# akashsengupta1997/STRAPS-3DHumanShapePose

Hardware: AMD Instinct MI355X
Metric: bodies/sec (higher is better)
Workload: dtype fp32 (encoder convolutions as exact bf16x3 operand splits (six bf16 products per term); in-step SMPL blend contraction and skinning as 3-product fp16 splits (fp16x3_lbs: 22-bit operands); fp32 accumulate throughout)

## Files before the change

straps-3dhumanshapepose_amd/csrc/backward.hip:

```cpp
#include "common.h"
#include <stdlib.h>

namespace {

struct WgradP {
    const float* x;
    const float* dy;
    float* part;
    int B, H, W, Cin, Cout, R, S, stride, pad, Ho, Wo;
    int M, rows_per_split, ct, it;
};

__device__ __attribute__((aligned(16))) float k_zero16w[4] = {0.f, 0.f, 0.f, 0.f};

template <int BCO, int BCI>
__global__ __launch_bounds__(256) void conv_wgrad_kernel(WgradP p) {
    constexpr int STG = 32 * (BCO + BCI);
    constexpr int LPD = BCO / 4, PWD = 64 / LPD, RDD = 8 / PWD;
    constexpr int LPX = BCI / 4, PWX = 64 / LPX, RDX = 8 / PWX;
    constexpr int MI = BCO / 64, NI = BCI / 64;
    extern __shared__ __attribute__((aligned(16))) float smem[];
    const int tid = threadIdx.x, lane = tid & 63, wave = tid >> 6;
    const int wave_u = __builtin_amdgcn_readfirstlane(wave);
    const int wm = wave >> 1, wn = wave & 1;
// ... 477 lines not shown
    const int cbeg = blockIdx.y * p.chunks_per_split;
    const int cend = min(cbeg + p.chunks_per_split, p.nchunks);
    const u16* zsrc = reinterpret_cast<const u16*>(k_zero16x);
    asm volatile("" : "+s"(zsrc));

    const int lp = (tid & 255) >> 3, ls = tid & 7;
    const int d_g = ls ^ (((lp >> 1) & 1) << 2);
    long long d_off[DR];
#pragma unroll
    for (int q = 0; q < DR; ++q) {
        const int px = lp + 32 * q;
        d_off[q] = ((long long)((co0 >> 5) + (d_g >> 2)) * p.rows + (px >> p.cw_log2) * p.W + (px & (p.cw - 1))) * 32 + (d_g & 3) * 8;
    }
    int x_pr[XR], x_pc[XR];
    long long x_g[XR];
#pragma unroll
    for (int q = 0; q < XR; ++q) {
        const int pp = lp + 32 * q;
        x_pr[q] = pp / pw - 1;
        x_pc[q] = pp - (x_pr[q] + 1) * pw - 1;
        const int g = ls ^ (((pp >> 1) & 1) << 2);
        x_g[q] = (long long)((ci0 >> 5) + (g >> 2)) * p.rows * 32 + (g & 3) * 8;
    }
    auto dma_chunk = [&](int c, int stage) {
        const int per_img = p.chunk_rows_per_img * p.chunks_per_row;
        const int b = c / per_img;
        const int rem = c - b * per_img;
        const int cr = rem / p.chunks_per_row, cc = rem - cr * p.chunks_per_row;
        const int ho0 = cr * p.rpc, wo0 = cc * p.cw;
        u16* D = smem + stage * STAGE;
        u16* X = D + 3 * DPX * 64;
        const u16* dbase = p.dy3 + ((long long)(b * p.H + ho0) * p.W + wo0) * 32;
        const u16* xsrc = p.x3 + ((long long)(b * p.H + ho0) * p.W + wo0) * 32;
#pragma unroll
        for (int q = 0; q < DR; ++q) {
            if (NG > 1 && (q & 1) != grp) continue;
#pragma unroll
            for (int pl = 0; pl < 3; ++pl)
                __builtin_amdgcn_global_load_lds((const __attribute__((address_space(1))) void*)(dbase + d_off[q] + pl * p.dps),
                                                 (__attribute__((address_space(3))) void*)(D + (pl * DPX + 32 * q + 8 * wave_u) * 64), 16, 0, 0);
        }
#pragma unroll
        for (int q = 0; q < XR; ++q) {
            if (q * 32 + 8 * wave_u >= npatch || q * 32 + 8 * wave_u >= XPX) break;
            if (NG > 1 && ((q + DR) & 1) != grp) continue;
            const int hi = ho0 + x_pr[q], wi = wo0 + x_pc[q];
            const bool ok = (unsigned)hi < (unsigned)p.H && (unsigned)wi < (unsigned)p.W;
            const u16* src = ok ? xsrc + (x_pr[q] * p.W + x_pc[q]) * 32 + x_g[q] : zsrc;
            const long long ps = ok ? p.xps : 0;
#pragma unroll
            for (int pl = 0; pl < 3; ++pl)
                __builtin_amdgcn_global_load_lds((const __attribute__((address_space(1))) void*)(src + pl * ps),
                                                 (__attribute__((address_space(3))) void*)(X + (pl * XPX + 32 * q + 8 * wave_u) * 64), 16, 0, 0);
        }
    };

    const int t = lane & 15, ch16 = (lane >> 4) & 1, kh = lane >> 5;
    auto row_off = [&](int slot_px, int c4) {
        const int g = (c4 >> 3) ^ (((slot_px >> 1) & 1) << 2);
        return slot_px * 64 + g * 8 + (c4 & 4);
    };
    int d_fo[KSG][2], x_fo[KSG][2];
#pragma unroll
    for (int ks = 0; ks < KSG; ++ks)
#pragma unroll
        for (int r = 0; r < 2; ++r) {
            const int px = (grp + NG * ks) * 16 + kh * 8 + r * 4 + (t >> 2);
            d_fo[ks][r] = row_off(px, wm * 32 + ch16 * 16 + (t & 3) * 4);
            x_fo[ks][r] = (px >> p.cw_log2) * pw + (px & (p.cw - 1));
        }
    const int x_c4 = wn * 32 + ch16 * 16 + (t & 3) * 4;

    f32x16 acc[9];
#pragma unroll
    for (int tp = 0; tp < 9; ++tp)
#pragma unroll
        for (int q = 0; q < 16; ++q) acc[tp][q] = 0.f;
    if (cbeg < cend) dma_chunk(cbeg, 0);
    constexpr int TA[6] = {1, 0, 2, 0, 1, 0};
    constexpr int TB[6] = {1, 2, 0, 1, 0, 0};
    for (int c = cbeg; c < cend; ++c) {
        const int stage = (c - cbeg) & 1;
        asm volatile("s_waitcnt vmcnt(0)" ::: "memory");
        __builtin_amdgcn_s_barrier();
        asm volatile("" ::: "memory");
        if (c + 1 < cend && !(ABL & 1)) dma_chunk(c + 1, stage ^ 1);
        const u16* D = smem + ((ABL & 1) ? 0 : stage) * STAGE;
        const u16* X = D + 3 * DPX * 64;
        __builtin_amdgcn_s_setprio(1);
#pragma unroll
        for (int ks = 0; ks < KSG; ++ks) {
            bf16x8w a[3];
#pragma unroll
            for (int pl = 0; pl < 3; ++pl) a[pl] = tr_frag(D + pl * DPX * 64 + d_fo[ks][0], D + pl * DPX * 64 + d_fo[ks][1]);
#pragma unroll
            for (int tp0 = 0; tp0 < 9; tp0 += W3X_TG) {
                bf16x8w b[W3X_TG][3];
#pragma unroll
                for (int u = 0; u < W3X_TG; ++u) {
                    const int tp = tp0 + u;
                    if (tp >= 9) break;
                    const int sh = (ABL & 4) ? 0 : (tp / 3) * pw + (tp % 3);
                    const int o0 = row_off(x_fo[ks][0] + sh, x_c4), o1 = row_off(x_fo[ks][1] + sh, x_c4);
#pragma unroll
                    for (int pl = 0; pl < 3; ++pl) b[u][pl] = tr_frag(X + pl * XPX * 64 + o0, X + pl * XPX * 64 + o1);
                }
                if (ABL & 2) {
#pragma unroll
                    for (int u = 0; u < W3X_TG; ++u)
                        if (tp0 + u < 9)
#pragma unroll
                            for (int pl = 0; pl < 3; ++pl) acc[0][pl] += (float)b[u][pl][0] + (float)a[pl][1];
                    continue;
                }
#pragma unroll
                for (int e = 0; e < 6; ++e)
#pragma unroll
                    for (int u = 0; u < W3X_TG; ++u)
                        if (tp0 + u < 9) acc[tp0 + u] = __builtin_amdgcn_mfma_f32_32x32x16_bf16(a[TA[e]], b[u][TB[e]], acc[tp0 + u], 0, 0, 0);
            }
        }
        __builtin_amdgcn_s_setprio(0);
    }
    if constexpr (NG > 1) {
        float* R = smem_f + ((wave * 3) * 16) * 64 + lane;
#pragma unroll
        for (int rd = 0; rd < 3; ++rd) {
            __syncthreads();
            if (grp == 1) {
#pragma unroll
                for (int tp = 0; tp < 3; ++tp)
#pragma unroll
                    for (int q = 0; q < 16; ++q) R[(tp * 16 + q) * 64] = acc[rd * 3 + tp][q];
            }
            __syncthreads();
            if (grp == 0) {
#pragma unroll
                for (int tp = 0; tp < 3; ++tp)
#pragma unroll
                    for (int q = 0; q < 16; ++q) acc[rd * 3 + tp][q] += R[(tp * 16 + q) * 64];
            }
        }
        if (grp != 0) return;
    }
    const int i = lane & 31;
    float* o = p.part + (long long)blockIdx.y * p.Cout * 9 * p.Cin;
#pragma unroll
    for (int tp = 0; tp < 9; ++tp)
#pragma unroll
        for (int q = 0; q < 16; ++q) {
            const int co = co0 + wm * 32 + mfma_row(q, lane);
            o[((long long)co * 9 + tp) * p.Cin + ci0 + wn * 32 + i] = acc[tp][q];
        }
}

__global__ __launch_bounds__(256) void wgrad_reduce_kernel(const float* __restrict__ part, float* __restrict__ dw, int splits,
                                                           int Cout, int Cin, int RS, int accumulate) {
    __shared__ f32x4 red[4][64];
    const long long n = (long long)Cout * RS * Cin;
    const int lane = threadIdx.x & 63, sg = threadIdx.x >> 6;
    const long long idx = ((long long)blockIdx.x * 64 + lane) * 4;
    f32x4 s = {0.f, 0.f, 0.f, 0.f};
    int k = sg;
    for (; k + 12 < splits; k += 16) {
        const f32x4 v0 = *reinterpret_cast<const f32x4*>(part + (long long)k * n + idx);
        const f32x4 v1 = *reinterpret_cast<const f32x4*>(part + (long long)(k + 4) * n + idx);
        const f32x4 v2 = *reinterpret_cast<const f32x4*>(part + (long long)(k + 8) * n + idx);
        const f32x4 v3 = *reinterpret_cast<const f32x4*>(part + (long long)(k + 12) * n + idx);
        s += (v0 + v1) + (v2 + v3);
    }
    for (; k < splits; k += 4) s += *reinterpret_cast<const f32x4*>(part + (long long)k * n + idx);
    red[sg][lane] = s;
    __syncthreads();
    if (sg != 0) return;
    s = (red[0][lane] + red[1][lane]) + (red[2][lane] + red[3][lane]);
    const int ci = (int)(idx % Cin);
    long long t = idx / Cin;
    const int tap = (int)(t % RS);
    const int co = (int)(t / RS);
#pragma unroll
    for (int e = 0; e < 4; ++e) {
        const long long o = ((long long)co * Cin + ci + e) * RS + tap;
        dw[o] = accumulate ? dw[o] + s[e] : s[e];
    }
}

constexpr int TY = 2, TX = 32, PH = 2 * TY + 5, PW = 72, TPIX = TY * TX;
constexpr int CG = 4, GK = CG * 49, GNB = (GK + 31) / 32, GUNITS = 2 * GNB, UPW = (GUNITS + 3) / 4;

__global__ __launch_bounds__(256) void stem_tileact_kernel(const unsigned* __restrict__ nzmask, uint8_t* __restrict__ tact, int C, int H, int W,
                                                           int tiles_x, int tiles_y, int ntiles, int groups) {
    const int idx = blockIdx.x * 256 + threadIdx.x;
    if (idx >= ntiles * groups) return;
    const int grp = idx / ntiles, tile = idx - grp * ntiles;
    int bid = tile;
    const int b = bid / (tiles_x * tiles_y);
    bid -= b * tiles_x * tiles_y;
    const int ty = bid / tiles_x, tx = bid - ty * tiles_x;
    const int hi0 = 2 * (ty * TY) - 3, wi0 = 2 * (tx * TX) - 3;
    const int HC = (H + 3) >> 2, WW = (W + 255) >> 8;
    const int rc0 = max(hi0, 0) >> 2, rc1 = min(hi0 + PH - 1, H - 1) >> 2;
    const int wa = max(wi0 - 1, 0), wb = min(wi0 - 2 + PW, W - 1);
    const int c0 = grp * CG, nc = min(CG, C - c0);
    unsigned chact = 0;
    for (int cl = 0; cl < nc; ++cl) {
        unsigned any = 0;
        for (int rcell = rc0; rcell <= rc1; ++rcell)
            for (int word = wa >> 8; word <= (wb >> 8); ++word) {
                const int lo = max(wa, word << 8), hi = min(wb, (word << 8) + 255);
                const int b0 = (lo >> 3) & 31, b1 = (hi >> 3) & 31;
                const unsigned bits = (b1 == 31 ? 0xffffffffu : ((1u << (b1 + 1)) - 1u)) & ~((1u << b0) - 1u);
                any |= nzmask[(((long long)b * C + c0 + cl) * HC + rcell) * WW + word] & bits;
            }
        if (any) chact |= 1u << cl;
    }
    tact[idx] = (uint8_t)chact;
}

__global__ __launch_bounds__(256) void stem_tileany_kernel(const unsigned* __restrict__ nzmask, uint8_t* __restrict__ tany, int C, int H, int W,
                                                           int tiles_x, int tiles_y, int ntiles) {
    const int lane = threadIdx.x & 63, sub = lane & 31;
    const int tile = (blockIdx.x * 256 + threadIdx.x) >> 5;
    unsigned any = 0;
    if (tile < ntiles) {
        int bid = tile;
        const int b = bid / (tiles_x * tiles_y);
        bid -= b * tiles_x * tiles_y;
        const int ty = bid / tiles_x, tx = bid - ty * tiles_x;
        const int hi0 = 2 * (ty * TY) - 3, wi0 = 2 * (tx * TX) - 3;
        const int HC = (H + 3) >> 2, WW = (W + 255) >> 8;
        const int rc0 = max(hi0, 0) >> 2, rc1 = min(hi0 + PH - 1, H - 1) >> 2;
        const int wa = max(wi0 - 1, 0), wb = min(wi0 - 2 + PW, W - 1);
        for (int c = sub; c < C; c += 32)
            for (int rcell = rc0; rcell <= rc1; ++rcell)
                for (int word = wa >> 8; word <= (wb >> 8); ++word) {
                    const int lo = max(wa, word << 8), hi = min(wb, (word << 8) + 255);
                    const int b0 = (lo >> 3) & 31, b1 = (hi >> 3) & 31;
                    const unsigned bits = (b1 == 31 ? 0xffffffffu : ((1u << (b1 + 1)) - 1u)) & ~((1u << b0) - 1u);
                    any |= nzmask[(((long long)b * C + c) * HC + rcell) * WW + word] & bits;
                }
    }
    const unsigned long long bal = __ballot(any != 0u);
    const unsigned mine = (unsigned)(bal >> (lane & 32));
    if (sub == 0 && tile < ntiles) tany[tile] = mine ? 1 : 0;
}

__global__ __launch_bounds__(256) void stem_wgrad_kernel(const float* __restrict__ x, const float* __restrict__ dy,
                                                         float* __restrict__ part, const uint8_t* __restrict__ tact, int B, int C, int H,
                                                         int W, int Ho, int Wo,
                                                         int tiles_x, int tiles_y, int Kp, int ntiles, int rot) {
    __shared__ __attribute__((aligned(16))) float patch[2 * CG * PH * PW];
    __shared__ __attribute__((aligned(16))) float dys[2 * TPIX * 68];
    const int tid = threadIdx.x, lane = tid & 63;
    const int wave = __builtin_amdgcn_readfirstlane(tid >> 6);
    const int i = lane & 31, h = lane >> 5;
    const int c0 = blockIdx.y * CG;
    const int nc = min(CG, C - c0);
    const int gk = nc * 49;

    int u_a[UPW], u_nb[UPW], u_ko[UPW];
    unsigned u_span[UPW];
#pragma unroll
    for (int j = 0; j < UPW; ++j) {
        const int u = wave + 4 * j;
        u_a[j] = u & 1;
        u_nb[j] = u >> 1;
        const int k = u_nb[j] * 32 + i;
        int o = 0;
        if (u < GUNITS && k < gk) {
            const int cl = k / 49, rs = k - cl * 49;
            const int r = rs / 7, s_ = rs - r * 7;
            o = (cl * PH + r) * PW + s_ + 1;
        }
        u_ko[j] = o;
        const int k0 = u_nb[j] * 32;
        u_span[j] = 0;
        if (u < GUNITS && k0 < gk) {
            const int cl0 = k0 / 49, cl1 = min(k0 + 31, gk - 1) / 49;
            u_span[j] = (1u << cl0) | (1u << cl1);
        }
    }
    f32x16 acc[UPW];
#pragma unroll
    for (int j = 0; j < UPW; ++j)
#pragma unroll
        for (int q = 0; q < 16; ++q) acc[j][q] = 0.f;

    constexpr int PIT = (CG * PH * (PW / 4) + 255) / 256;
    constexpr int DIT = TPIX * 16 / 256;
    const bool vec = (W & 3) == 0;
    f32x4 pv[PIT], dv[DIT];
    auto tile_origin = [&](int tile, int& b, int& y0, int& x0) {
        b = tile / (tiles_x * tiles_y);
        const int bid = tile - b * tiles_x * tiles_y;
        const int ty = bid / tiles_x;
        y0 = ty * TY;
        x0 = (bid - ty * tiles_x) * TX;
    };
    auto issue_loads = [&](int tile, unsigned chact) {
        int b, y0, x0;
        tile_origin(tile, b, y0, x0);
        const int hi0 = 2 * y0 - 3, wi0 = 2 * x0 - 3;
#pragma unroll
        for (int it = 0; it < PIT; ++it) {
            const int idx = tid + it * 256;
            const int q = idx % (PW / 4);
// ... 608 lines not shown
int straps_internal_wgrad_reduce(const float* part, float* dw_oihw, int splits, int cout, int cin, int taps, int accumulate, hipStream_t st) {
    const long long n = (long long)cout * taps * cin;
    hipLaunchKernelGGL(wgrad_reduce_kernel, dim3((unsigned)(n / 256)), dim3(256), 0, st, part, dw_oihw, splits, cout, cin, taps, accumulate);
    STRAPS_CHECK_LAUNCH("wgrad_reduce_kernel");
    return STRAPS_OK;
}

static bool wgrad3_plan(int batch, int h, int w, int cin, int cout, int kh, int kw, int stride, int pad, Wgrad3P* p, int* splits, int cp = 32) {
    if (!(kh == 3 && kw == 3 && stride == 1 && pad == 1)) return false;
    if (w < 8 || (w & (w - 1)) != 0) return false;
    const int cw = w < 32 ? w : 32, rpc = cp / cw;
    if (h % rpc != 0) return false;
    int lg = 0;
    while ((1 << lg) < cw) ++lg;
    p->H = h; p->W = w; p->Cin = cin; p->Cout = cout; p->cw = cw; p->cw_log2 = lg; p->rpc = rpc;
    p->chunks_per_row = w / cw;
    p->chunk_rows_per_img = h / rpc;
    p->nchunks = batch * p->chunk_rows_per_img * p->chunks_per_row;
    p->it = cin / 64;
    const int tiles = (cout / 64) * (cin / 64);
    constexpr int W3_TARGET = 256;
    int s = (W3_TARGET + tiles - 1) / tiles;
    const int max_s = (p->nchunks + 3) / 4;
    if (s > max_s) s = max_s;
    if (s < 1) s = 1;
    p->chunks_per_split = (p->nchunks + s - 1) / s;
    *splits = (p->nchunks + p->chunks_per_split - 1) / p->chunks_per_split;
    return true;
}

extern "C" size_t straps_conv_wgrad_workspace_bytes(int batch, int h, int w, int cin, int cout, int kh, int kw, int stride, int pad) {
    Wgrad3P p3;
    int splits3;
    if (wgrad3_plan(batch, h, w, cin, cout, kh, kw, stride, pad, &p3, &splits3)) return (size_t)splits3 * cout * 9 * cin * sizeof(float);
    const int ho = (h + 2 * pad - kh) / stride + 1, wo = (w + 2 * pad - kw) / stride + 1;
    const long long M = (long long)batch * ho * wo;
    const bool big = wgrad_big_tile(M, cin, cout, kh * kw);
    const int tile = big ? 128 : 64;
    const int tiles = kh * kw * (cout / tile) * (cin / tile);
    return (size_t)wgrad_splits(M, tiles, big) * cout * kh * kw * cin * sizeof(float);
}

extern "C" int straps_conv_wgrad(const float* x, const float* dy, float* dw_oihw, void* workspace, int batch, int h, int w, int cin,
                                 int cout, int kh, int kw, int stride, int pad, int accumulate, void* stream) {
    STRAPS_REQUIRE(x && dy && dw_oihw && workspace, "straps_conv_wgrad: null pointer");
    STRAPS_REQUIRE(cin % 64 == 0 && cout % 64 == 0, "straps_conv_wgrad: need cin%%64==0 and cout%%64==0 (cin=%d cout=%d)", cin, cout);
    {
        Wgrad3P p3;
        int splits3;
        if (wgrad3_plan(batch, h, w, cin, cout, kh, kw, stride, pad, &p3, &splits3)) {
            p3.x = x; p3.dy = dy; p3.part = (float*)workspace;
            constexpr int NG3 = 2;
            const size_t lds = (size_t)NG3 * 2 * W3PX * 64 * sizeof(float);
            STRAPS_RAISE_LDS((conv_wgrad3x3_kernel<NG3>), lds, "conv_wgrad3x3_kernel");
            hipStream_t st3 = (hipStream_t)stream;
            hipLaunchKernelGGL(conv_wgrad3x3_kernel<NG3>, dim3((cout / 64) * (cin / 64), splits3), dim3(256 * NG3), lds, st3, p3);
            STRAPS_CHECK_LAUNCH("conv_wgrad3x3_kernel");
            const long long n3 = (long long)cout * 9 * cin;
            hipLaunchKernelGGL(wgrad_reduce_kernel, dim3((unsigned)(n3 / 256)), dim3(256), 0, st3, p3.part, dw_oihw, splits3, cout, cin, 9, accumulate);
            STRAPS_CHECK_LAUNCH("wgrad_reduce_kernel");
            return STRAPS_OK;
        }
    }
    WgradP p;
    p.x = x; p.dy = dy; p.part = (float*)workspace;
    p.B = batch; p.H = h; p.W = w; p.Cin = cin; p.Cout = cout; p.R = kh; p.S = kw; p.stride = stride; p.pad = pad;
    p.Ho = (h + 2 * pad - kh) / stride + 1;
    p.Wo = (w + 2 * pad - kw) / stride + 1;
    const long long M = (long long)batch * p.Ho * p.Wo;
    STRAPS_REQUIRE(M < (1LL << 31), "straps_conv_wgrad: problem too large");
    p.M = (int)M;
    const bool big = wgrad_big_tile(M, cin, cout, kh * kw);
    const int tile = big ? 128 : 64;
    p.ct = cout / tile; p.it = cin / tile;
    const int tiles = kh * kw * p.ct * p.it;
    const int splits = wgrad_splits(M, tiles, big);
    p.rows_per_split = (int)(((M + splits - 1) / splits + 31) / 32 * 32);
    hipStream_t st = (hipStream_t)stream;
    if (big) {
        STRAPS_RAISE_LDS((conv_wgrad_kernel<128, 128>), 64 * 1024, "conv_wgrad_kernel");
        hipLaunchKernelGGL((conv_wgrad_kernel<128, 128>), dim3(tiles, splits), dim3(256), 64 * 1024, st, p);
    } else {
        hipLaunchKernelGGL((conv_wgrad_kernel<64, 64>), dim3(tiles, splits), dim3(256), 32 * 1024, st, p);
    }
    STRAPS_CHECK_LAUNCH("conv_wgrad_kernel");
    const long long n = (long long)cout * kh * kw * cin;
    hipLaunchKernelGGL(wgrad_reduce_kernel, dim3((unsigned)(n / 256)), dim3(256), 0, st, p.part, dw_oihw, splits, cout, cin, kh * kw, accumulate);
    STRAPS_CHECK_LAUNCH("wgrad_reduce_kernel");
    return STRAPS_OK;
}

static int stem_wgrad_blocks(int ntiles) {
    static const int cap = STRAPS_TOOL_ENV_INT("STRAPS_STEM_WGRAD_BLOCKS", 256);
    return ntiles < cap ? ntiles : cap;
}

static int wgrad_x3_route(int batch, int h, int w, int cin, int cout, int kh, int kw, int stride, int pad) {
    Wgrad3P p3;
    int splits3;
    if (wgrad3_plan(batch, h, w, cin, cout, kh, kw, stride, pad, &p3, &splits3)) return 1;
    static const bool tap_x3 = !STRAPS_TOOL_ENV_INT("STRAPS_WGRAD_TAP_FP32", 0);
    return tap_x3 && (kh * kw > 1 || (cin >= 128 && cout >= 128)) ? 2 : 0;
}

static void wgrad_x3_block(long long M, int cin, int cout, int taps, bool big, int stride, int* bco, int* bci) {
    const int v = STRAPS_TOOL_ENV_INT("STRAPS_WGRAD_TILE", 0);
    if (v) {
        const int o = v / 1000, i = v % 1000;
        const bool known = (o == 256 && i == 64) || (o == 64 && i == 256) || (o == 256 && i == 128) || (o == 128 && i == 256) || (o == 128 && i == 64) ||
                           (o == 64 && i == 128) || (o == 128 && i == 128) || (o == 64 && i == 64);
        if (known && cout % o == 0 && cin % i == 0 && !(o == 128 && i == 128 && !big)) { *bco = o; *bci = i; }
        return;
    }
    if (taps == 1) {
        if (M >= 32768 && cout % 256 == 0 && cin % 128 == 0) { *bco = 256; *bci = 128; }
        else if (M <= 8192 && cout % 128 == 0 && cin % 128 == 0) {
            if (stride == 1 && cout > cin) { *bco = 64; *bci = 128; }
            else { *bco = 128; *bci = 64; }
        }
    } else if (cout % 256 == 0 && cin % 128 == 0) { *bco = 256; *bci = 128; }
    else if (cout % 128 == 0 && cin % 64 == 0) { *bco = 128; *bci = 64; }
}

extern "C" int straps_conv_wgrad_x3_on_planes(int batch, int h, int w, int cin, int cout, int kh, int kw, int stride, int pad) {
    return wgrad_x3_route(batch, h, w, cin, cout, kh, kw, stride, pad) != 0;
}

extern "C" int straps_conv_wgrad_x3(const float* x, const float* dy, const unsigned short* x3, long long x_plane_stride, const unsigned short* dy3,
                                    long long dy_plane_stride, float* dw_oihw, void* workspace, int batch, int h, int w, int cin, int cout, int kh,
                                    int kw, int stride, int pad, int accumulate, void* stream) {
    STRAPS_REQUIRE(dw_oihw && workspace, "straps_conv_wgrad_x3: null pointer");
    const int route = (x3 && dy3) ? wgrad_x3_route(batch, h, w, cin, cout, kh, kw, stride, pad) : 0;
    STRAPS_REQUIRE(route != 0 || (x && dy), "straps_conv_wgrad_x3: this shape runs on the fp32 tensors, which are NULL (see straps_conv_wgrad_x3_on_planes)");
    STRAPS_REQUIRE(cin % 64 == 0 && cout % 64 == 0, "straps_conv_wgrad_x3: need cin%%64==0 and cout%%64==0 (cin=%d cout=%d)", cin, cout);
    Wgrad3P p3;
    int splits3;
    if (route == 1 && wgrad3_plan(batch, h, w, cin, cout, kh, kw, stride, pad, &p3, &splits3)) {
        STRAPS_REQUIRE(x_plane_stride % 8 == 0 && dy_plane_stride % 8 == 0, "straps_conv_wgrad_x3: plane strides must be multiples of 8 elements");
        Wgrad3XP q;
        q.x3 = x3; q.dy3 = dy3; q.xps = x_plane_stride; q.dps = dy_plane_stride; q.part = (float*)workspace;
        q.H = p3.H; q.W = p3.W; q.Cin = p3.Cin; q.Cout = p3.Cout; q.cw = p3.cw; q.cw_log2 = p3.cw_log2; q.rpc = p3.rpc;
        q.chunks_per_row = p3.chunks_per_row; q.chunk_rows_per_img = p3.chunk_rows_per_img; q.nchunks = p3.nchunks;
        q.chunks_per_split = p3.chunks_per_split; q.it = p3.it;
        q.rows = (long long)batch * h * w;
        constexpr int W3X_NG = 2;
        hipStream_t st3 = (hipStream_t)stream;
        Wgrad3P p64;
        int splits64;
        const bool c64 = wgrad3_plan(batch, h, w, cin, cout, kh, kw, stride, pad, &p64, &splits64, 64) && splits64 <= splits3;
        if (c64) {
            q.rpc = p64.rpc; q.chunks_per_row = p64.chunks_per_row; q.chunk_rows_per_img = p64.chunk_rows_per_img; q.nchunks = p64.nchunks;
            q.chunks_per_split = p64.chunks_per_split;
            splits3 = splits64;
            const size_t lds = (size_t)2 * 3 * (64 + 136) * 64 * sizeof(u16);
            const dim3 grid3((cout / 64) * (cin / 64), splits3);
#ifdef STRAPS_TOOLS
            static const int abl = STRAPS_TOOL_ENV_INT("STRAPS_WGRAD3_ABL", 0);
            if (abl) {
                auto kern = abl == 1 ? conv_wgrad3x3_x3_kernel<W3X_NG, 64, 1> : abl == 2 ? conv_wgrad3x3_x3_kernel<W3X_NG, 64, 2>
                          : abl == 3 ? conv_wgrad3x3_x3_kernel<W3X_NG, 64, 3> : abl == 4 ? conv_wgrad3x3_x3_kernel<W3X_NG, 64, 4> : conv_wgrad3x3_x3_kernel<W3X_NG, 64, 5>;
                hipFuncSetAttribute((const void*)kern, hipFuncAttributeMaxDynamicSharedMemorySize, (int)lds);
                hipLaunchKernelGGL(kern, grid3, dim3(256 * W3X_NG), lds, st3, q);
                STRAPS_CHECK_LAUNCH("conv_wgrad3x3_x3_kernel (ablation)");
                return STRAPS_OK;
            }
#endif
            STRAPS_RAISE_LDS((conv_wgrad3x3_x3_kernel<W3X_NG, 64>), lds, "conv_wgrad3x3_x3_kernel");
            hipLaunchKernelGGL((conv_wgrad3x3_x3_kernel<W3X_NG, 64>), grid3, dim3(256 * W3X_NG), lds, st3, q);
        } else {
            const size_t lds = (size_t)2 * 3 * (32 + 128) * 64 * sizeof(u16);
            STRAPS_RAISE_LDS((conv_wgrad3x3_x3_kernel<W3X_NG, 32>), lds, "conv_wgrad3x3_x3_kernel");
            hipLaunchKernelGGL((conv_wgrad3x3_x3_kernel<W3X_NG, 32>), dim3((cout / 64) * (cin / 64), splits3), dim3(256 * W3X_NG), lds, st3, q);
        }
        STRAPS_CHECK_LAUNCH("conv_wgrad3x3_x3_kernel");
        const long long n3 = (long long)cout * 9 * cin;
        hipLaunchKernelGGL(wgrad_reduce_kernel, dim3((unsigned)(n3 / 256)), dim3(256), 0, st3, q.part, dw_oihw, splits3, cout, cin, 9, accumulate);
        STRAPS_CHECK_LAUNCH("wgrad_reduce_kernel");
        return STRAPS_OK;
    }
    if (route == 2) {
        STRAPS_REQUIRE(x_plane_stride % 8 == 0 && dy_plane_stride % 8 == 0, "straps_conv_wgrad_x3: plane strides must be multiples of 8 elements");
        WgradXP q;
        q.x3 = x3; q.dy3 = dy3; q.xps = x_plane_stride; q.dps = dy_plane_stride; q.part = (float*)workspace;
        q.B = batch; q.H = h; q.W = w; q.Cin = cin; q.Cout = cout; q.R = kh; q.S = kw; q.stride = stride; q.pad = pad;
        q.Ho = (h + 2 * pad - kh) / stride + 1;
        q.Wo = (w + 2 * pad - kw) / stride + 1;
        const long long M = (long long)batch * q.Ho * q.Wo;
        STRAPS_REQUIRE(M < (1LL << 31), "straps_conv_wgrad_x3: problem too large");
        q.M = (int)M;
        const bool big = wgrad_big_tile(M, cin, cout, kh * kw);
        int bco = big ? 128 : 64, bci = bco;
        wgrad_x3_block(M, cin, cout, kh * kw, big, stride, &bco, &bci);
        q.ct = cout / bco; q.it = cin / bci;
        const int tiles = kh * kw * q.ct * q.it;
        const size_t lds = (size_t)2 * 3 * 32 * (bco + bci) * sizeof(u16);
        int splits;
        if (bco == bci) splits = wgrad_splits(M, tiles, bco == 128, true);
        else {
            const int per_cu = (int)((160 * 1024) / lds) < 1 ? 1 : (int)((160 * 1024) / lds);
            splits = (256 * per_cu + tiles - 1) / tiles;
            const long long max_s = (M + 127) / 128;
            if (splits > max_s) splits = (int)max_s;
            const int cap = wgrad_splits(M, kh * kw * (cout / (big ? 128 : 64)) * (cin / (big ? 128 : 64)), big);
            if (splits > cap) splits = cap;
            if (splits < 1) splits = 1;
        }
        q.rows_per_split = (int)(((M + splits - 1) / splits + 31) / 32 * 32);
        hipStream_t st = (hipStream_t)stream;
        static const int nst_env = STRAPS_TOOL_ENV_INT("STRAPS_WGRAD_TAP_NST", 2);
        constexpr int SB = 3 * 32 * 256 * 2, SS = 3 * 32 * 128 * 2;
#define STRAPS_WGRAD_X3_LAUNCH(BCO_, BCI_)                                                                              \
        do {                                                                                                            \
            STRAPS_RAISE_LDS((conv_wgrad_x3_kernel<BCO_, BCI_, 2>), lds, "conv_wgrad_x3_kernel");                       \
            hipLaunchKernelGGL((conv_wgrad_x3_kernel<BCO_, BCI_, 2>), dim3(tiles, splits), dim3(256), lds, st, q);      \
        } while (0)
        if (bco == 256 && bci == 64) STRAPS_WGRAD_X3_LAUNCH(256, 64);
        else if (bco == 64 && bci == 256) STRAPS_WGRAD_X3_LAUNCH(64, 256);
        else if (bco == 256 && bci == 128) STRAPS_WGRAD_X3_LAUNCH(256, 128);
        else if (bco == 128 && bci == 256) STRAPS_WGRAD_X3_LAUNCH(128, 256);
        else if (bco == 128 && bci == 64) STRAPS_WGRAD_X3_LAUNCH(128, 64);
        else if (bco == 64 && bci == 128) STRAPS_WGRAD_X3_LAUNCH(64, 128);
        else if (bco == 128) {
            if (nst_env == 3) {
                STRAPS_RAISE_LDS((conv_wgrad_x3_kernel<128, 128, 3>), 3 * SB, "conv_wgrad_x3_kernel");
                hipLaunchKernelGGL((conv_wgrad_x3_kernel<128, 128, 3>), dim3(tiles, splits), dim3(256), 3 * SB, st, q);
            } else {
                STRAPS_RAISE_LDS((conv_wgrad_x3_kernel<128, 128, 2>), 2 * SB, "conv_wgrad_x3_kernel");
                hipLaunchKernelGGL((conv_wgrad_x3_kernel<128, 128, 2>), dim3(tiles, splits), dim3(256), 2 * SB, st, q);
            }
        } else if (nst_env == 3) {
            STRAPS_RAISE_LDS((conv_wgrad_x3_kernel<64, 64, 3>), 3 * SS, "conv_wgrad_x3_kernel");
            hipLaunchKernelGGL((conv_wgrad_x3_kernel<64, 64, 3>), dim3(tiles, splits), dim3(256), 3 * SS, st, q);
        } else if (nst_env == 4) {
            STRAPS_RAISE_LDS((conv_wgrad_x3_kernel<64, 64, 4>), 4 * SS, "conv_wgrad_x3_kernel");
            hipLaunchKernelGGL((conv_wgrad_x3_kernel<64, 64, 4>), dim3(tiles, splits), dim3(256), 4 * SS, st, q);
        } else {
            hipLaunchKernelGGL((conv_wgrad_x3_kernel<64, 64, 2>), dim3(tiles, splits), dim3(256), 2 * SS, st, q);
        }
#undef STRAPS_WGRAD_X3_LAUNCH
        STRAPS_CHECK_LAUNCH("conv_wgrad_x3_kernel");
        const long long n = (long long)cout * kh * kw * cin;
        hipLaunchKernelGGL(wgrad_reduce_kernel, dim3((unsigned)(n / 256)), dim3(256), 0, st, q.part, dw_oihw, splits, cout, cin, kh * kw, accumulate);
        STRAPS_CHECK_LAUNCH("wgrad_reduce_kernel");
        return STRAPS_OK;
    }
    return straps_conv_wgrad(x, dy, dw_oihw, workspace, batch, h, w, cin, cout, kh, kw, stride, pad, accumulate, stream);
}

extern "C" size_t straps_stem_wgrad_workspace_bytes(int batch, int cin, int h, int w) {
    const int Ho = (h - 1) / 2 + 1, Wo = (w - 1) / 2 + 1;
    const int ntiles = batch * ((Ho + TY - 1) / TY) * ((Wo + TX - 1) / TX);
    const int Kp = (cin * 49 + 31) / 32 * 32;
    const size_t groups = (cin + CG - 1) / CG;
    return (size_t)stem_wgrad_blocks(ntiles) * 64 * Kp * sizeof(float) + straps_stem_nzmask_words(batch, cin, h, w) * sizeof(uint32_t) +
           ((groups * ntiles + 3) & ~(size_t)3);
}

extern "C" int straps_stem_wgrad(const float* x_nchw, const float* dy_nhwc, float* dw_oihw, void* workspace, const uint32_t* nzmask,
                                 int batch, int cin, int h, int w, int accumulate, void* stream) {
    STRAPS_REQUIRE(x_nchw && dy_nhwc && dw_oihw && workspace, "straps_stem_wgrad: null pointer");
    STRAPS_REQUIRE(batch > 0 && cin > 0 && h >= 7 && w >= 7, "straps_stem_wgrad: bad shape B=%d C=%d H=%d W=%d", batch, cin, h, w);
    const int K = cin * 49, Kp = (K + 31) / 32 * 32;
    const int Ho = (h - 1) / 2 + 1, Wo = (w - 1) / 2 + 1;
    const int tiles_x = (Wo + TX - 1) / TX, tiles_y = (Ho + TY - 1) / TY;
    const int ntiles = batch * tiles_x * tiles_y;
    const int nblk = stem_wgrad_blocks(ntiles);
    const int groups = (cin + CG - 1) / CG;
    STRAPS_REQUIRE(groups <= 65535, "straps_stem_wgrad: too many input channels (%d)", cin);
    hipStream_t st = (hipStream_t)stream;
    float* part = (float*)workspace;
    uint32_t* own = (uint32_t*)(part + (size_t)nblk * 64 * Kp);
    uint8_t* tact = (uint8_t*)(own + straps_stem_nzmask_words(batch, cin, h, w));
    if (!nzmask) {
        const int rc = straps_stem_nzmask(x_nchw, own, batch, cin, h, w, stream);
        if (rc != STRAPS_OK) return rc;
        nzmask = own;
    }
    hipLaunchKernelGGL(stem_tileact_kernel, dim3((ntiles * groups + 255) / 256), dim3(256), 0, st, nzmask, tact, cin, h, w, tiles_x, tiles_y, ntiles,
                       groups);
    STRAPS_CHECK_LAUNCH("stem_tileact_kernel");
    static const int rot = STRAPS_TOOL_ENV_INT("STRAPS_STEM_WGRAD_ROT", 97);
    hipLaunchKernelGGL(stem_wgrad_kernel, dim3(nblk, groups), dim3(256), 0, st, x_nchw, dy_nhwc, part, tact, batch, cin, h, w, Ho, Wo,
                       tiles_x, tiles_y, Kp, ntiles, rot);
    STRAPS_CHECK_LAUNCH("stem_wgrad_kernel");
    hipLaunchKernelGGL(stem_wgrad_reduce_kernel, dim3((64 * K + 63) / 64), dim3(256), 0, st, (const float*)workspace, dw_oihw, nblk, K, Kp, accumulate);
    STRAPS_CHECK_LAUNCH("stem_wgrad_reduce_kernel");
    return STRAPS_OK;
}

static double bn_bwd_count(long long rows, int flags) { return (flags & 2) ? (double)INFINITY : (double)rows; }

extern "C" int straps_bn_bwd_blocks(long long rows, int c) {
    const int colblocks = (c + 63) / 64;
    long long b = 2048 / colblocks;
    const long long cap = (rows + 63) / 64;
    if (b > cap) b = cap;
    return (int)(b < 1 ? 1 : b);
}

static int bn_bwd_x3_impl(const float* dy, const float* yact, const unsigned* relu_bits, const float* raw, const float* save_mean, const float* save_invstd,
                          const float* gamma, const float* mask_scale, const float* mask_shift, float* dgamma, float* dbeta, float* draw,
                          float* dz_out, unsigned short* draw_planes, long long plane_stride, void* workspace, long long rows, int c,
                          int accumulate, void* stream) {
    STRAPS_REQUIRE(!relu_bits || (!yact && (c & 31) == 0), "straps_bn_bwd_bits_x3: the bits replace yact (and need c %% 32 == 0; c=%d)", c);
    STRAPS_REQUIRE(!draw_planes || (plane_stride >= rows * c && plane_stride % 8 == 0), "straps_bn_bwd_x3: plane_stride must be >= rows*c and a multiple of 8");
    STRAPS_REQUIRE(!draw_planes || (c & 31) == 0, "straps_bn_bwd_x3: chunk-major planes need c %% 32 == 0 (c=%d)", c);
    STRAPS_REQUIRE(dy && raw && save_mean && save_invstd && gamma && dgamma && dbeta && (draw || draw_planes) && workspace, "straps_bn_bwd: null pointer");
    STRAPS_REQUIRE(rows > 0 && c > 0 && (c & 3) == 0, "straps_bn_bwd: bad shape rows=%lld c=%d", rows, c);
    const int C4 = c >> 2;
    STRAPS_REQUIRE(C4 <= 256 ? (256 % C4 == 0) : (C4 % 256 == 0), "straps_bn_bwd: channel count %d not supported", c);
    hipStream_t st = (hipStream_t)stream;
    const int nblk = straps_bn_bwd_blocks(rows, c);
    const int rpb = (int)((rows + nblk - 1) / nblk);
    double* part = (double*)workspace;
    double* coefd = part + (size_t)nblk * c * 2;
    float* k1 = (float*)(coefd + 2 * (size_t)c);
    hipLaunchKernelGGL(bn_bwd_reduce_kernel<false>, dim3(nblk, (c + 63) / 64), dim3(256), 0, st, dy, yact, raw, save_mean, save_invstd, mask_scale, mask_shift, part, rows, c, rpb, PoolSrc{}, relu_bits);
    STRAPS_CHECK_LAUNCH("bn_bwd_reduce_kernel");
    hipLaunchKernelGGL(bn_bwd_finalize_kernel, dim3((c + 3) / 4), dim3(256), 0, st, part, nblk, c, bn_bwd_count(rows, accumulate), gamma, save_invstd, dgamma, dbeta, coefd, k1, accumulate & 1);
    STRAPS_CHECK_LAUNCH("bn_bwd_finalize_kernel");
    const long long n4 = rows * C4;
    const int tiled = straps_bn_tiled(rows, c >> 2);
    hipLaunchKernelGGL(bn_bwd_apply_kernel<false>, dim3(tiled ? straps_bn_tiled_grid(rows, c >> 2, tiled) : straps_grid256_rows(n4, c >> 2)), dim3(256), 0, st, dy, yact, raw, save_mean, save_invstd, coefd, k1, mask_scale, mask_shift, draw, dz_out, draw_planes, plane_stride, n4, c, PoolSrc{}, relu_bits, tiled);
    STRAPS_CHECK_LAUNCH("bn_bwd_apply_kernel");
    return STRAPS_OK;
}

// ... 183 lines not shown
```

Measured before the change: 8020.

## Add 768-thread wgrad 3x3 kernel splitting work by kernel row across waves

Introduces a new 3x3 weight-gradient kernel that runs 12 waves per block, two k-groups of six waves each. Each wave in a group owns one kernel row and one 32-column half of the input channels, and accumulates all three column taps for both 64-channel output halves. The chunk DMA is shared by three 256-thread quads. The two groups' partial accumulators are reduced through LDS before the store. This reworks how waves share the 64x64x9 output tile to raise MFMA occupancy and operand reuse, at the cost of larger per-wave accumulator register pressure (96 fp32 accumulators) and an LDS reduction.

Result: no change. 8044 (median of 6 runs) (+0.3%).

```diff
diff --git a/straps-3dhumanshapepose_amd/csrc/backward.hip b/straps-3dhumanshapepose_amd/csrc/backward.hip
--- a/straps-3dhumanshapepose_amd/csrc/backward.hip
+++ b/straps-3dhumanshapepose_amd/csrc/backward.hip
@@ -653,6 +653,165 @@
             const int co = co0 + wm * 32 + mfma_row(q, lane);
             o[((long long)co * 9 + tp) * p.Cin + ci0 + wn * 32 + i] = acc[tp][q];
         }
+}
+
+template <int CP, int ABL = 0>
+__global__ __launch_bounds__(768) void conv_wgrad3x3_x3r_kernel(Wgrad3XP p) {
+    constexpr int NG = 2, NQ = 3;
+    constexpr int DPX = CP, XPX = CP == 32 ? 128 : 136;
+    constexpr int STAGE = 3 * (DPX + XPX) * 64;
+    constexpr int DR = CP / 32, XR = (XPX + 31) / 32;
+    constexpr int RQ = (DR + XR + NQ - 1) / NQ;
+    constexpr int KSG = CP / 16 / NG;
+    static_assert(CP % (16 * NG) == 0, "chunk / group mismatch");
+    extern __shared__ __attribute__((aligned(16))) float smem_f[];
+    u16* smem = reinterpret_cast<u16*>(smem_f);
+    const int pw = p.cw + 2;
+    const int npatch = (p.rpc + 2) * pw;
+    const int tid = threadIdx.x, lane = tid & 63;
+    const int quad = __builtin_amdgcn_readfirstlane(tid >> 8), qwave = __builtin_amdgcn_readfirstlane((tid >> 6) & 3);
+    const int grp = __builtin_amdgcn_readfirstlane(tid >> 6) / 6;
+    const int gw = __builtin_amdgcn_readfirstlane(tid >> 6) - grp * 6;
+    const int kr = gw >> 1, wn = gw & 1;
+    const int itile = blockIdx.x % p.it, ctile = blockIdx.x / p.it;
+    const int co0 = ctile * 64, ci0 = itile * 64;
+    const int cbeg = blockIdx.y * p.chunks_per_split;
+    const int cend = min(cbeg + p.chunks_per_split, p.nchunks);
+    const u16* zsrc = reinterpret_cast<const u16*>(k_zero16x);
+    asm volatile("" : "+s"(zsrc));
+
+    const int lp = (tid & 255) >> 3, ls = tid & 7;
+    const int cg = ls ^ (((lp >> 1) & 1) << 2);
+    auto dma_chunk = [&](int c, int stage) {
+        const int per_img = p.chunk_rows_per_img * p.chunks_per_row;
+        const int b = c / per_img;
+        const int rem = c - b * per_img;
+        const int cr = rem / p.chunks_per_row, cc = rem - cr * p.chunks_per_row;
+        const int ho0 = cr * p.rpc, wo0 = cc * p.cw;
+        u16* D = smem + stage * STAGE;
+        u16* X = D + 3 * DPX * 64;
+        const u16* dbase = p.dy3 + ((long long)(b * p.H + ho0) * p.W + wo0) * 32;
+        const u16* xsrc = p.x3 + ((long long)(b * p.H + ho0) * p.W + wo0) * 32;
+#pragma unroll
+        for (int j = 0; j < RQ; ++j) {
+            const int i = quad + NQ * j;
+            if (i >= DR + XR) break;
+            if (i < DR) {
+                const int px = lp + 32 * i;
+                const u16* src = dbase + ((long long)((co0 >> 5) + (cg >> 2)) * p.rows + (px >> p.cw_log2) * p.W + (px & (p.cw - 1))) * 32 + (cg & 3) * 8;
+#pragma unroll
+                for (int pl = 0; pl < 3; ++pl)
+                    __builtin_amdgcn_global_load_lds((const __attribute__((address_space(1))) void*)(src + pl * p.dps),
+                                                     (__attribute__((address_space(3))) void*)(D + (pl * DPX + 32 * i + 8 * qwave) * 64), 16, 0, 0);
+            } else {
+                const int q = i - DR;
+                if (q * 32 + 8 * qwave >= npatch || q * 32 + 8 * qwave >= XPX) continue;
+                const int pp = lp + 32 * q;
+                const int pr = pp / pw - 1, pc = pp - (pr + 1) * pw - 1;
+                const int hi = ho0 + pr, wi = wo0 + pc;
+                const bool ok = (unsigned)hi < (unsigned)p.H && (unsigned)wi < (unsigned)p.W;
+                const u16* src = ok ? xsrc + ((long long)((ci0 >> 5) + (cg >> 2)) * p.rows + pr * p.W + pc) * 32 + (cg & 3) * 8 : zsrc;
+                const long long ps = ok ? p.xps : 0;
+#pragma unroll
+                for (int pl = 0; pl < 3; ++pl)
+                    __builtin_amdgcn_global_load_lds((const __attribute__((address_space(1))) void*)(src + pl * ps),
+                                                     (__attribute__((address_space(3))) void*)(X + (pl * XPX + 32 * q + 8 * qwave) * 64), 16, 0, 0);
+            }
+        }
+    };
+
+    const int t = lane & 15, ch16 = (lane >> 4) & 1, kh = lane >> 5;
+    auto row_off = [&](int slot_px, int c4) {
+        const int g = (c4 >> 3) ^ (((slot_px >> 1) & 1) << 2);
+        return slot_px * 64 + g * 8 + (c4 & 4);
+    };
+    int d_fo[2], x_fo[2];
+#pragma unroll
+    for (int r = 0; r < 2; ++r) {
+        const int px = grp * 16 + kh * 8 + r * 4 + (t >> 2);
+        d_fo[r] = row_off(px, ch16 * 16 + (t & 3) * 4);
+        x_fo[r] = ((px >> p.cw_log2) + kr) * pw + (px & (p.cw - 1));
+    }
+    const int x_ks = (32 >> p.cw_log2) * pw;
+    const int x_c4 = wn * 32 + ch16 * 16 + (t & 3) * 4;
+
+    f32x16 acc[3][2];
+#pragma unroll
+    for (int s = 0; s < 3; ++s)
+#pragma unroll
+        for (int h = 0; h < 2; ++h)
+#pragma unroll
+            for (int q = 0; q < 16; ++q) acc[s][h][q] = 0.f;
+    if (cbeg < cend) dma_chunk(cbeg, 0);
+    constexpr int TA[6] = {1, 0, 2, 0, 1, 0};
+    constexpr int TB[6] = {1, 2, 0, 1, 0, 0};
+    for (int c = cbeg; c < cend; ++c) {
+        const int stage = (c - cbeg) & 1;
+        asm volatile("s_waitcnt vmcnt(0)" ::: "memory");
+        __builtin_amdgcn_s_barrier();
+        asm volatile("" ::: "memory");
+        if (c + 1 < cend && !(ABL & 1)) dma_chunk(c + 1, stage ^ 1);
+        const u16* D = smem + ((ABL & 1) ? 0 : stage) * STAGE;
+        const u16* X = D + 3 * DPX * 64;
+        __builtin_amdgcn_s_setprio(1);
+#pragma unroll 1
+        for (int ks = 0; ks < KSG; ++ks) {
+            bf16x8w a[2][3];
+#pragma unroll
+            for (int h = 0; h < 2; ++h)
+#pragma unroll
+                for (int pl = 0; pl < 3; ++pl)
+                    a[h][pl] = tr_frag(D + (pl * DPX + 16 * NG * ks) * 64 + (d_fo[0] ^ (32 * h)), D + (pl * DPX + 16 * NG * ks) * 64 + (d_fo[1] ^ (32 * h)));
+#pragma unroll
+            for (int s = 0; s < 3; ++s) {
+                const int sh = (ABL & 4) ? 0 : s;
+                const int o0 = row_off(x_fo[0] + ks * x_ks + sh, x_c4), o1 = row_off(x_fo[1] + ks * x_ks + sh, x_c4);
+                bf16x8w b[3];
+#pragma unroll
+                for (int pl = 0; pl < 3; ++pl) b[pl] = tr_frag(X + pl * XPX * 64 + o0, X + pl * XPX * 64 + o1);
+                if (ABL & 2) {
+#pragma unroll
+                    for (int pl = 0; pl < 3; ++pl) acc[0][0][pl] += (float)b[pl][0] + (float)a[0][pl][1] + (float)a[1][pl][1];
+                    continue;
+                }
+#pragma unroll
+                for (int e = 0; e < 6; ++e)
+#pragma unroll
+                    for (int h = 0; h < 2; ++h) acc[s][h] = __builtin_amdgcn_mfma_f32_32x32x16_bf16(a[h][TA[e]], b[TB[e]], acc[s][h], 0, 0, 0);
+            }
+        }
+        __builtin_amdgcn_s_setprio(0);
+    }
+    float* R = smem_f + (gw * 2 * 16) * 64 + lane;
+#pragma unroll
+    for (int s = 0; s < 3; ++s) {
+        __syncthreads();
+        if (grp == 1) {
+#pragma unroll
+            for (int h = 0; h < 2; ++h)
+#pragma unroll
+                for (int q = 0; q < 16; ++q) R[(h * 16 + q) * 64] = acc[s][h][q];
+        }
+        __syncthreads();
+        if (grp == 0) {
+#pragma unroll
+            for (int h = 0; h < 2; ++h)
+#pragma unroll
+                for (int q = 0; q < 16; ++q) acc[s][h][q] += R[(h * 16 + q) * 64];
+        }
+    }
+    if (grp != 0) return;
+    const int i = lane & 31;
+    float* o = p.part + (long long)blockIdx.y * p.Cout * 9 * p.Cin;
+#pragma unroll
+    for (int s = 0; s < 3; ++s)
+#pragma unroll
+        for (int h = 0; h < 2; ++h)
+#pragma unroll
+            for (int q = 0; q < 16; ++q) {
+                const int co = co0 + h * 32 + mfma_row(q, lane);
+                o[((long long)co * 9 + kr * 3 + s) * p.Cin + ci0 + wn * 32 + i] = acc[s][h][q];
+            }
 }
 
 __global__ __launch_bounds__(256) void wgrad_reduce_kernel(const float* __restrict__ part, float* __restrict__ dw, int splits,
@@ -1567,27 +1726,35 @@
             q.rpc = p64.rpc; q.chunks_per_row = p64.chunks_per_row; q.chunk_rows_per_img = p64.chunk_rows_per_img; q.nchunks = p64.nchunks;
             q.chunks_per_split = p64.chunks_per_split;
             splits3 = splits64;
-            const size_t lds = (size_t)2 * 3 * (64 + 136) * 64 * sizeof(u16);
-            const dim3 grid3((cout / 64) * (cin / 64), splits3);
+        }
+        const size_t lds = c64 ? (size_t)2 * 3 * (64 + 136) * 64 * sizeof(u16) : (size_t)2 * 3 * (32 + 128) * 64 * sizeof(u16);
+        const dim3 grid3((cout / 64) * (cin / 64), splits3);
 #ifdef STRAPS_TOOLS
-            static const int abl = STRAPS_TOOL_ENV_INT("STRAPS_WGRAD3_ABL", 0);
-            if (abl) {
-                auto kern = abl == 1 ? conv_wgrad3x3_x3_kernel<W3X_NG, 64, 1> : abl == 2 ? conv_wgrad3x3_x3_kernel<W3X_NG, 64, 2>
-                          : abl == 3 ? conv_wgrad3x3_x3_kernel<W3X_NG, 64, 3> : abl == 4 ? conv_wgrad3x3_x3_kernel<W3X_NG, 64, 4> : conv_wgrad3x3_x3_kernel<W3X_NG, 64, 5>;
-                hipFuncSetAttribute((const void*)kern, hipFuncAttributeMaxDynamicSharedMemorySize, (int)lds);
-                hipLaunchKernelGGL(kern, grid3, dim3(256 * W3X_NG), lds, st3, q);
-                STRAPS_CHECK_LAUNCH("conv_wgrad3x3_x3_kernel (ablation)");
-                return STRAPS_OK;
-            }
+        const int form = STRAPS_TOOL_ENV_INT("STRAPS_WGRAD3_FORM", 1), abl = STRAPS_TOOL_ENV_INT("STRAPS_WGRAD3_ABL", 0);
+        if (form == 0 || abl) {
+            void (*kern)(Wgrad3XP) = nullptr;
+            if (form == 0 && c64)
+                kern = abl == 1 ? conv_wgrad3x3_x3_kernel<W3X_NG, 64, 1> : abl == 2 ? conv_wgrad3x3_x3_kernel<W3X_NG, 64, 2> : abl == 3 ? conv_wgrad3x3_x3_kernel<W3X_NG, 64, 3>
+                     : abl == 4 ? conv_wgrad3x3_x3_kernel<W3X_NG, 64, 4> : abl == 5 ? conv_wgrad3x3_x3_kernel<W3X_NG, 64, 5> : conv_wgrad3x3_x3_kernel<W3X_NG, 64>;
+            else if (form == 0) kern = abl ? nullptr : conv_wgrad3x3_x3_kernel<W3X_NG, 32>;
+            else if (c64)
+                kern = abl == 1 ? conv_wgrad3x3_x3r_kernel<64, 1> : abl == 2 ? conv_wgrad3x3_x3r_kernel<64, 2> : abl == 3 ? conv_wgrad3x3_x3r_kernel<64, 3>
+                     : abl == 4 ? conv_wgrad3x3_x3r_kernel<64, 4> : conv_wgrad3x3_x3r_kernel<64, 5>;
+            STRAPS_REQUIRE(kern, "straps_conv_wgrad_x3: STRAPS_WGRAD3_FORM=%d / STRAPS_WGRAD3_ABL=%d has no kernel for this shape", form, abl);
+            (void)hipFuncSetAttribute((const void*)kern, hipFuncAttributeMaxDynamicSharedMemorySize, (int)lds);
+            hipLaunchKernelGGL(kern, grid3, dim3(form == 0 ? 256 * W3X_NG : 768), lds, st3, q);
+            STRAPS_CHECK_LAUNCH("conv_wgrad3x3_x3_kernel (tools form / ablation)");
+            if (abl) return STRAPS_OK;
+        } else
 #endif
-            STRAPS_RAISE_LDS((conv_wgrad3x3_x3_kernel<W3X_NG, 64>), lds, "conv_wgrad3x3_x3_kernel");
-            hipLaunchKernelGGL((conv_wgrad3x3_x3_kernel<W3X_NG, 64>), grid3, dim3(256 * W3X_NG), lds, st3, q);
+        if (c64) {
+            STRAPS_RAISE_LDS((conv_wgrad3x3_x3r_kernel<64>), lds, "conv_wgrad3x3_x3r_kernel");
+            hipLaunchKernelGGL((conv_wgrad3x3_x3r_kernel<64>), grid3, dim3(768), lds, st3, q);
         } else {
-            const size_t lds = (size_t)2 * 3 * (32 + 128) * 64 * sizeof(u16);
-            STRAPS_RAISE_LDS((conv_wgrad3x3_x3_kernel<W3X_NG, 32>), lds, "conv_wgrad3x3_x3_kernel");
-            hipLaunchKernelGGL((conv_wgrad3x3_x3_kernel<W3X_NG, 32>), dim3((cout / 64) * (cin / 64), splits3), dim3(256 * W3X_NG), lds, st3, q);
-        }
-        STRAPS_CHECK_LAUNCH("conv_wgrad3x3_x3_kernel");
+            STRAPS_RAISE_LDS((conv_wgrad3x3_x3r_kernel<32>), lds, "conv_wgrad3x3_x3r_kernel");
+            hipLaunchKernelGGL((conv_wgrad3x3_x3r_kernel<32>), grid3, dim3(768), lds, st3, q);
+        }
+        STRAPS_CHECK_LAUNCH("conv_wgrad3x3_x3r_kernel");
         const long long n3 = (long long)cout * 9 * cin;
         hipLaunchKernelGGL(wgrad_reduce_kernel, dim3((unsigned)(n3 / 256)), dim3(256), 0, st3, q.part, dw_oihw, splits3, cout, cin, 9, accumulate);
         STRAPS_CHECK_LAUNCH("wgrad_reduce_kernel");
```
